# ChrisTho23/DrakeGPT

Hardware: AMD Instinct MI355X
Metric: training tokens/sec (fwd+bwd+AdamW) (higher is better)
Workload: dtype bf16; 1 GPU; TransformerLM_scaled: V=80 C=384 T=256 heads=6 layers=6 dropout=0.2; fwd+bwd+AdamW; hipGraph=on; batch_per_gpu=64, global_batch=64, seq_len=256, parallelism=dp1, dp_gradient_buckets=1, params=10800464

## Files before the change

drakegpt_amd/csrc/chain.hip:

```cpp
#include "common.h"
#include <stdlib.h>

typedef __attribute__((address_space(1))) const void* gptr_t;
typedef __attribute__((address_space(3))) void* lptr_t;

#define CH_C 384
#define CH_ROWS 64
#define CH_STAGE_B 24576
#define CH_STAGE_A 4096
#define CH_STAGE (CH_STAGE_B + CH_STAGE_A)
#define CH_NST 4
#define CH_ARES (CH_NST * CH_STAGE)
#define CH_KS (CH_C / 32)

struct ChainP {
    const char* o;
    const float* x;
    const char* wproj; const float* bproj;
    float* x1;
    const float* ln2w; const float* ln2b; float* mean2; float* rstd2; bf16_t* h2;
    const char* w1; const float* b1; bf16_t* f; unsigned char* bits;
    const char* w2; const float* b2;
    float* x2; bf16_t* x2b;
    const float* ln1w; const float* ln1b; float* mean1; float* rstd1; bf16_t* h1;
    const char* wqkv; bf16_t* qkv;
    int M, n_blocks;
    float eps;
    const uint32_t* rng; uint32_t site_proj, site_ffn, thr; float inv_keep; int drop;
    int stagger;
    unsigned long long* stamps;
    int dbg;
};

__device__ __forceinline__ void ch_wait_vm(int n) {
    switch (n) {
        case 6: asm volatile("s_waitcnt vmcnt(6)" ::: "memory"); break;
        case 7: asm volatile("s_waitcnt vmcnt(7)" ::: "memory"); break;
        case 12: asm volatile("s_waitcnt vmcnt(12)" ::: "memory"); break;
        case 13: asm volatile("s_waitcnt vmcnt(13)" ::: "memory"); break;
        case 14: asm volatile("s_waitcnt vmcnt(14)" ::: "memory"); break;
        case 8: asm volatile("s_waitcnt vmcnt(8)" ::: "memory"); break;
        case 18: asm volatile("s_waitcnt vmcnt(18)" ::: "memory"); break;
        case 20: asm volatile("s_waitcnt vmcnt(20)" ::: "memory"); break;
        default: asm volatile("s_waitcnt vmcnt(0)" ::: "memory"); break;
    }
}

template <int MODE>
__global__ __launch_bounds__(768) void block_chain_fwd_kernel(ChainP p) {
    constexpr int C = CH_C, KS = CH_KS;
    constexpr bool HAS_PROJ = MODE == 0 || MODE == 1 || MODE == 3, HAS_FFN1 = MODE == 0 || MODE == 1;
    constexpr bool HAS_FFN2 = MODE == 0 || MODE == 1 || MODE == 4, HAS_QKV = MODE == 0 || MODE == 2;
    constexpr bool LN_FFN2 = MODE == 0 || MODE == 4;
    constexpr int O_FFN1 = HAS_PROJ ? KS : 0, O_FFN2 = O_FFN1 + (HAS_FFN1 ? 4 * KS : 0), Q0 = O_FFN2 + (HAS_FFN2 ? 4 * KS : 0);
    constexpr int S = Q0 + (HAS_QKV ? 3 * KS : 0);
    __shared__ __attribute__((aligned(16))) char lds[CH_ARES + 6 * 8192];
    const int tid = threadIdx.x, lane = tid & 63, wave = __builtin_amdgcn_readfirstlane(tid >> 6);
    const bool loader = wave >= 8;
    if (p.stagger > 0) {
        const int grp = ((int)blockIdx.x >> 3) & 3;
        for (int i = 0; i < grp * p.stagger; ++i) __builtin_amdgcn_s_sleep(1);
    }

    auto n_of = [&](int s) -> int {
        if (MODE == 4) return (s & 1) ? 6 : 8;
        return (HAS_FFN2 && s >= O_FFN2 && s < Q0) ? 7 : 6;
    };
    auto ln_after = [&](int s) -> bool { return (HAS_PROJ && s == O_FFN1 - 1) || (LN_FFN2 && s == Q0 - 1); };

    if (loader) {
        const int lw = wave - 8;
        const int prow = lane >> 3, slot = lane & 7;
        const int ls = slot ^ prow;
        const uint32_t voff = (uint32_t)(lw * 6144 + lane * 16);
        const uint32_t aoff = (uint32_t)((lw * 8 + prow + 32 * (ls >> 2)) * (4 * C * 2) + (ls & 3) * 16);
        for (int blk = blockIdx.x; blk < p.n_blocks; blk += gridDim.x) {
            const int64_t row0 = (int64_t)blk * CH_ROWS;
            const char* fblk = (const char*)p.f + row0 * (int64_t)(4 * C * 2);
            auto issue = [&](int s) {
                if (p.dbg == 3 && s >= CH_NST) return;
                const char* src;
                if (HAS_PROJ && s < O_FFN1) src = p.wproj + (int64_t)s * CH_STAGE_B;
                else if (HAS_FFN1 && s < O_FFN2) src = p.w1 + (int64_t)(s - O_FFN1) * CH_STAGE_B;
                else if (HAS_FFN2 && s < Q0) src = p.w2 + (int64_t)(s - O_FFN2) * CH_STAGE_B;
                else src = p.wqkv + (int64_t)(s - Q0) * CH_STAGE_B;
                char* buf = lds + (s & (CH_NST - 1)) * CH_STAGE;
#pragma unroll
                for (int i = 0; i < 6; ++i)
                    __builtin_amdgcn_global_load_lds((gptr_t)(src + voff + i * 1024), (lptr_t)(buf + lw * 6144 + i * 1024), 16, 0, 0);
                if (MODE == 4) {
                    if (!(s & 1)) {
                        const int u = s >> 1;
#pragma unroll
                        for (int j = 0; j < 2; ++j) {
                            const int pr = lw * 2 + j;
                            const char* src = fblk + (int64_t)(pr * 8 + prow) * (4 * C * 2) + u * 128 + ((slot ^ prow) << 4);
                            __builtin_amdgcn_global_load_lds((gptr_t)src, (lptr_t)(lds + CH_ARES + (u % 6) * 8192 + pr * 1024), 16, 0, 0);
                        }
                    }
                } else if (HAS_FFN2 && s >= O_FFN2 && s < Q0)
                    __builtin_amdgcn_global_load_lds((gptr_t)(fblk + (s - O_FFN2) * 64 + aoff), (lptr_t)(buf + CH_STAGE_B + lw * 1024), 16, 0, 0);
            };
            if (HAS_PROJ) {
                const int chunk_std = slot ^ prow;
#pragma unroll
                for (int j = 0; j < 12; ++j) {
                    const int idx = lw * 12 + j, tile = idx >> 3, pr = idx & 7;
                    const char* src = p.o + (row0 + pr * 8 + prow) * (int64_t)(C * 2) + tile * 128 + chunk_std * 16;
                    __builtin_amdgcn_global_load_lds((gptr_t)src, (lptr_t)(lds + CH_ARES + tile * 8192 + pr * 1024), 16, 0, 0);
                }
            }
            for (int s = 0; s < CH_NST; ++s) issue(s);
            if (MODE == 2) __builtin_amdgcn_s_barrier();
            ch_wait_vm(n_of(1) + n_of(2) + n_of(3));
            __builtin_amdgcn_s_barrier();
            if (p.dbg == 5) {
                for (int b = 0; b + 1 < S; ++b) {
                    __builtin_amdgcn_s_barrier();
                    if (ln_after(b)) __builtin_amdgcn_s_barrier();
                }
                if (ln_after(S - 1)) __builtin_amdgcn_s_barrier();
                __builtin_amdgcn_s_barrier();
                continue;
            }
            for (int b = 0; b + 1 < S; ++b) {
                int fly = 0;
                if (b + 2 < S) fly += n_of(b + 2);
                if (b + 3 < S) fly += n_of(b + 3);
                ch_wait_vm(fly);
                __builtin_amdgcn_s_barrier();
                if (b + CH_NST < S) issue(b + CH_NST);
                if (ln_after(b)) __builtin_amdgcn_s_barrier();
            }
            if (ln_after(S - 1)) __builtin_amdgcn_s_barrier();
            __builtin_amdgcn_s_barrier();
        }
        return;
    }

    const int wm = wave >> 2, wn = wave & 3;
    const int fr = lane & 15, fg = lane >> 4;
    f32x4 acc[2][6];
#pragma unroll
    for (int i = 0; i < 2; ++i)
#pragma unroll
        for (int j = 0; j < 6; ++j) acc[i][j] = (f32x4){0.f, 0.f, 0.f, 0.f};
    const int b_off = ((wn & 1) * 96 + fr) * 128 + ((((wn >> 1) * 4 + fg) ^ (fr & 7)) << 4);
    const int ar_off = CH_STAGE_B + fr * 128 + (((wm * 4 + fg) ^ (fr & 7)) << 4);
    const int res_row = wm * 32 + fr;
    const int a_off0 = CH_ARES + res_row * 128 + (((0 + fg) ^ (fr & 7)) << 4);
    const int a_off1 = CH_ARES + res_row * 128 + (((4 + fg) ^ (fr & 7)) << 4);
    auto read_B = [&](u32x4 (&fb)[6], int s) {
        const char* buf = lds + (s & (CH_NST - 1)) * CH_STAGE + b_off;
#pragma unroll
        for (int j = 0; j < 6; ++j) fb[j] = *(const u32x4*)(buf + j * 2048);
    };
    auto read_A_ring = [&](u32x4 (&fa)[2], int s) {
        const char* buf = lds + (s & (CH_NST - 1)) * CH_STAGE + ar_off;
#pragma unroll
        for (int i = 0; i < 2; ++i) fa[i] = *(const u32x4*)(buf + i * 2048);
    };
    auto read_A_res = [&](u32x4 (&fa)[2], int t) {
        const char* buf = lds + ((t >> 1) % 6) * 8192 + ((t & 1) ? a_off1 : a_off0);
#pragma unroll
        for (int i = 0; i < 2; ++i) fa[i] = *(const u32x4*)(buf + i * 2048);
    };
    auto mma = [&](const u32x4 (&fa)[2], const u32x4 (&fb)[6]) {
        if (p.dbg == 2) return;
#pragma unroll
        for (int i = 0; i < 2; ++i)
#pragma unroll
            for (int j = 0; j < 6; ++j)
                acc[i][j] = __builtin_amdgcn_mfma_f32_16x16x32_bf16(__builtin_bit_cast(bf16x8, fb[j]), __builtin_bit_cast(bf16x8, fa[i]), acc[i][j], 0, 0, 0);
    };
    uint32_t key_proj = 0, key_ffn = 0;
    if (p.drop) { key_proj = dg_site_key_dev(p.rng, p.site_proj); key_ffn = dg_site_key_dev(p.rng, p.site_ffn); }
    const int col_l = wn * 96 + (fg & 1) * 16 + (fg >> 1) * 8;
    auto opaque_lane = [&]() -> int { int l = lane; asm volatile("" : "+v"(l)); return l; };
    auto mad24 = [](int a, int b, int c) -> int { int r; asm("v_mad_u32_u24 %0, %1, %2, %3" : "=v"(r) : "v"(a), "s"(b), "v"(c)); return r; };

    auto take = [&](int i, int q, float (&v)[8]) {
#pragma unroll
        for (int e = 0; e < 4; ++e) {
            float a = acc[i][2 * q][e], b = acc[i][2 * q + 1][e];
            asm volatile("s_nop 1\n\tv_permlane16_swap_b32 %0, %1\n\ts_nop 1" : "+v"(a), "+v"(b));
            v[e] = a;
            v[4 + e] = b;
        }
        acc[i][2 * q] = (f32x4){0.f, 0.f, 0.f, 0.f};
        acc[i][2 * q + 1] = (f32x4){0.f, 0.f, 0.f, 0.f};
    };
    auto drop8 = [&](float (&v)[8], uint32_t key, int64_t row0, int rl, int col) {
        const uint32_t i0 = (uint32_t)row0 * (uint32_t)C + (uint32_t)mad24(rl, C, col);
        const uint32_t w2 = (i0 >> 1) * DG_WEYL;
#pragma unroll
        for (int e = 0; e < 8; e += 2) {
            const uint32_t h = dg_hash_w(key, w2 + (uint32_t)(e >> 1) * DG_WEYL);
            v[e] = dg_keep_lo(h, p.thr) ? v[e] * p.inv_keep : 0.f;
            v[e + 1] = dg_keep_hi(h, p.thr) ? v[e + 1] * p.inv_keep : 0.f;
        }
    };
    auto layernorm = [&](float (&xv)[2][3][8], float* scratch, int64_t row0, const float* gamma, const float* beta, float* mean_o,
                         float* rstd_o, bf16_t* y) {
        const int lo = opaque_lane(), fr = lo & 15, fg = lo >> 4, col_l = wn * 96 + (fg & 1) * 16 + (fg >> 1) * 8;
#pragma unroll
        for (int i = 0; i < 2; ++i) {
            float s = 0.f;
#pragma unroll
            for (int q = 0; q < 3; ++q)
#pragma unroll
                for (int e = 0; e < 8; ++e) s += xv[i][q][e];
            s += __shfl_xor(s, 16, 64);
            s += __shfl_xor(s, 32, 64);
            const float mw = s * (1.f / 96.f);
            float m2 = 0.f;
#pragma unroll
            for (int q = 0; q < 3; ++q)
#pragma unroll
                for (int e = 0; e < 8; ++e) { const float d = xv[i][q][e] - mw; m2 += d * d; }
            m2 += __shfl_xor(m2, 16, 64);
            m2 += __shfl_xor(m2, 32, 64);
            if (fg == 0) *(f32x2*)(scratch + ((wm * 32 + i * 16 + fr) * 4 + wn) * 2) = (f32x2){mw, m2};
        }
        __builtin_amdgcn_s_barrier();
        float mu[2], rs[2];
#pragma unroll
        for (int i = 0; i < 2; ++i) {
            const f32x4 a = *(const f32x4*)(scratch + (wm * 32 + i * 16 + fr) * 8), b = *(const f32x4*)(scratch + (wm * 32 + i * 16 + fr) * 8 + 4);
            const float m = ((a[0] + a[2]) + (b[0] + b[2])) * 0.25f;
            const float d0 = a[0] - m, d1 = a[2] - m, d2 = b[0] - m, d3 = b[2] - m;
            const float M2 = ((a[1] + a[3]) + (b[1] + b[3])) + 96.f * ((d0 * d0 + d1 * d1) + (d2 * d2 + d3 * d3));
            mu[i] = m;
            rs[i] = rsqrtf(M2 * (1.f / (float)C) + p.eps);
            if (wn == 0 && fg == 0) { mean_o[row0 + wm * 32 + i * 16 + fr] = m; rstd_o[row0 + wm * 32 + i * 16 + fr] = rs[i]; }
        }
#pragma unroll
        for (int q = 0; q < 3; ++q) {
            const int col = col_l + 32 * q;
            const f32x4 g0 = *(const f32x4*)(gamma + col), g1 = *(const f32x4*)(gamma + col + 4);
            const f32x4 b0 = *(const f32x4*)(beta + col), b1 = *(const f32x4*)(beta + col + 4);
#pragma unroll
            for (int i = 0; i < 2; ++i) {
                bf16x8 o;
#pragma unroll
                for (int e = 0; e < 4; ++e) {
                    o[e] = (bf16_t)((xv[i][q][e] - mu[i]) * rs[i] * g0[e] + b0[e]);
                    o[4 + e] = (bf16_t)((xv[i][q][4 + e] - mu[i]) * rs[i] * g1[e] + b1[e]);
                }
                const int rl = wm * 32 + i * 16 + fr;
                if (p.dbg != 6) *(bf16x8*)(y + row0 * C + mad24(rl, C, col)) = o;
                *(bf16x8*)(lds + CH_ARES + (col >> 6) * 8192 + rl * 128 + ((((col & 63) >> 3) ^ (rl & 7)) << 4)) = o;
            }
        }
    };
    auto residual_epilogue = [&](float (&xv)[2][3][8], int64_t row0, const float* bias, const float* res, uint32_t key, float* out32, bf16_t* out16) {
        const int lo = opaque_lane(), fr = lo & 15, fg = lo >> 4, col_l = wn * 96 + (fg & 1) * 16 + (fg >> 1) * 8;
        f32x4 bq[2][2], r[2][2][2];
        auto request = [&](int q) {
            const int col = col_l + 32 * q;
            bq[q & 1][0] = *(const f32x4*)(bias + col); bq[q & 1][1] = *(const f32x4*)(bias + col + 4);
#pragma unroll
            for (int i = 0; i < 2; ++i) {
                const float* rp = res + row0 * C + mad24(wm * 32 + i * 16 + fr, C, col);
                if (p.dbg == 7) { r[q & 1][i][0] = bq[q & 1][0]; r[q & 1][i][1] = bq[q & 1][1]; continue; }
                r[q & 1][i][0] = *(const f32x4*)rp; r[q & 1][i][1] = *(const f32x4*)(rp + 4);
            }
        };
        request(0);
#pragma unroll
        for (int q = 0; q < 3; ++q) {
            if (q + 1 < 3) request(q + 1);
            const int col = col_l + 32 * q;
#pragma unroll
            for (int i = 0; i < 2; ++i) {
                const int64_t row = row0 + wm * 32 + i * 16 + fr;
                float v[8];
                take(i, q, v);
#pragma unroll
                for (int e = 0; e < 4; ++e) { v[e] += bq[q & 1][0][e]; v[4 + e] += bq[q & 1][1][e]; }
                if (p.drop) drop8(v, key, row0, wm * 32 + i * 16 + fr, col);
#pragma unroll
                for (int e = 0; e < 4; ++e) { v[e] += r[q & 1][i][0][e]; v[4 + e] += r[q & 1][i][1][e]; }
                if (p.dbg == 6) {
                } else if (out32) {
                    float* op = out32 + row0 * C + mad24(wm * 32 + i * 16 + fr, C, col);
                    *(f32x4*)op = (f32x4){v[0], v[1], v[2], v[3]};
                    *(f32x4*)(op + 4) = (f32x4){v[4], v[5], v[6], v[7]};
                } else {
                    bf16x8 o;
#pragma unroll
                    for (int e = 0; e < 8; ++e) o[e] = (bf16_t)v[e];
                    *(bf16x8*)(out16 + row0 * C + mad24(wm * 32 + i * 16 + fr, C, col)) = o;
                }
#pragma unroll
                for (int e = 0; e < 8; ++e) xv[i][q][e] = v[e];
            }
        }
    };

    if (p.dbg != 11) {
        const int jx = (int)blockIdx.x >> 3, per = ((int)gridDim.x >> 3) ? ((int)gridDim.x >> 3) : 1;
        float w0 = 0.f, w1 = 0.f, w2 = 0.f, w3 = 0.f;
        auto warm = [&](float& dst, const char* base, int n_stages) {
            const int i = jx + per * tid;
            if (i < n_stages * (CH_STAGE_B / 128)) asm volatile("global_load_dword %0, %1, off" : "=v"(dst) : "v"(base + (int64_t)i * 128) : "memory");
        };
        if (HAS_PROJ) warm(w0, p.wproj, KS);
        if (HAS_FFN1) warm(w1, p.w1, 4 * KS);
        if (HAS_FFN2) warm(w2, p.w2, 4 * KS);
        if (HAS_QKV) warm(w3, p.wqkv, 3 * KS);
        asm volatile("s_waitcnt vmcnt(0)" : "+v"(w0), "+v"(w1), "+v"(w2), "+v"(w3) :: "memory");
    }
    auto stamp = [&](int k) {
        if (p.stamps && wave == 0) {
            const unsigned long long t = __builtin_amdgcn_s_memtime();
            if (lane == 0) p.stamps[(int64_t)blockIdx.x * 24 + k] = t;
        }
    };
    u32x4 fa0[2], fb0[6], fa1[2], fb1[6];
    for (int blk = blockIdx.x; blk < p.n_blocks; blk += gridDim.x) {
        const int64_t row0 = (int64_t)blk * CH_ROWS;
        int g = 0;
        if (MODE == 2) {
            float xv[2][3][8];
#pragma unroll
            for (int q = 0; q < 3; ++q)
#pragma unroll
                for (int i = 0; i < 2; ++i) {
                    const float* xp = p.x + row0 * C + mad24(wm * 32 + i * 16 + fr, C, col_l + 32 * q);
                    const f32x4 a = *(const f32x4*)xp, b = *(const f32x4*)(xp + 4);
#pragma unroll
                    for (int e = 0; e < 4; ++e) { xv[i][q][e] = a[e]; xv[i][q][4 + e] = b[e]; }
                }
            layernorm(xv, (float*)(lds + 0 * CH_STAGE + CH_STAGE_B), row0, p.ln1w, p.ln1b, p.mean1, p.rstd1, p.h1);
        }
        __builtin_amdgcn_s_barrier();
        auto pipe_barrier = [&]() {
            __builtin_amdgcn_sched_barrier(0);
            asm volatile("s_waitcnt lgkmcnt(0)" ::: "memory");
            __builtin_amdgcn_s_barrier();
            __builtin_amdgcn_sched_barrier(0);
        };
        auto piece = [&](int nstep, bool ring_a, bool next, bool a_after_barrier, bool drain = false) {
            read_B(fb0, g);
            if (!a_after_barrier) { if (ring_a) read_A_ring(fa0, g); else read_A_res(fa0, 0); }
            for (int t = 0; t < nstep; t += 2) {
                if (drain && t == nstep - 2 && p.dbg != 10) asm volatile("s_waitcnt vmcnt(0)" ::: "memory");
                if (t == 8) asm volatile("s_waitcnt vmcnt(0)" ::: "memory");
                pipe_barrier();
                if (t == 0 && a_after_barrier) read_A_res(fa0, 0);
                read_B(fb1, g + 1);
                if (ring_a) read_A_ring(fa1, g + 1); else read_A_res(fa1, t + 1);
                mma(fa0, fb0);
                ++g;
                if (t + 2 < nstep) {
                    pipe_barrier();
                    read_B(fb0, g + 1);
                    if (ring_a) read_A_ring(fa0, g + 1); else read_A_res(fa0, t + 2);
                } else if (next) {
                    pipe_barrier();
                }
                mma(fa1, fb1);
                ++g;
            }
            __builtin_amdgcn_sched_barrier(0);
            asm volatile("s_nop 15\n\ts_nop 3" ::: "memory");
            __builtin_amdgcn_sched_barrier(0);
        };
        stamp(0);
        if (HAS_PROJ) {
            piece(KS, false, HAS_FFN1, false, true);
            stamp(1);
            if (p.dbg == 4 || p.dbg == 5) __builtin_amdgcn_s_barrier();
            else {
                float xv[2][3][8];
                residual_epilogue(xv, row0, p.bproj, p.x, key_proj, p.x1, nullptr);
                layernorm(xv, (float*)(lds + (g & (CH_NST - 1)) * CH_STAGE + CH_STAGE_B), row0, p.ln2w, p.ln2b, p.mean2, p.rstd2, p.h2);
            }
        }
        stamp(2);
        if (HAS_FFN1) {
            for (int c = 0; c < 4; ++c) {
                piece(KS, false, true, c == 0);
                stamp(3 + 2 * c);
                if (p.dbg == 4 || p.dbg == 5) continue;
                const int lo = opaque_lane(), fr = lo & 15, fg = lo >> 4, col_l = wn * 96 + (fg & 1) * 16 + (fg >> 1) * 8;
                const int lane = lo;
                const int tile_lo = (blk >> 1) * (4 * C / 192) + c * 2 + (wn >> 1);
                const int wv = (((blk & 1) * 2 + wm) * 2 + (wn & 1));
                f32x4 bq[3][2];
#pragma unroll
                for (int q = 0; q < 3; ++q) {
                    const int col = c * C + col_l + 32 * q;
                    bq[q][0] = *(const f32x4*)(p.b1 + col); bq[q][1] = *(const f32x4*)(p.b1 + col + 4);
                }
#pragma unroll
                for (int q = 0; q < 3; ++q) {
                    const int col = c * C + col_l + 32 * q;
#pragma unroll
                    for (int i = 0; i < 2; ++i) {
                        const int64_t row = row0 + wm * 32 + i * 16 + fr;
                        float v[8];
                        take(i, q, v);
                        unsigned bm = 0;
                        bf16x8 o;
#pragma unroll
                        for (int e = 0; e < 8; ++e) {
                            v[e] = fmaxf(v[e] + (e < 4 ? bq[q][0][e] : bq[q][1][e - 4]), 0.f);
                            bm |= (v[e] > 0.f ? 1u : 0u) << e;
                            o[e] = (bf16_t)v[e];
                        }
                        if (p.dbg != 6) {
                            p.bits[((((int64_t)tile_lo * 8 + wv) * 3 + q) * 2 + i) * 64 + lane] = (unsigned char)bm;
                            *(bf16x8*)(p.f + row0 * (4 * C) + mad24(wm * 32 + i * 16 + fr, 4 * C, col)) = o;
                        }
                    }
                }
                stamp(4 + 2 * c);
            }
        }
        if (HAS_FFN2) {
            piece(4 * KS, MODE != 4, HAS_QKV, false, true);
            stamp(11);
            if (p.dbg == 4 || p.dbg == 5) { if (LN_FFN2) __builtin_amdgcn_s_barrier(); }
            else {
                float xv[2][3][8];
                residual_epilogue(xv, row0, p.b2, p.x1, key_ffn, MODE != 1 ? p.x2 : nullptr, p.x2b);
                if (LN_FFN2)
                    layernorm(xv, (float*)(lds + (g & (CH_NST - 1)) * CH_STAGE + CH_STAGE_B), row0, p.ln1w, p.ln1b, p.mean1, p.rstd1, p.h1);
            }
        }
        stamp(12);
        if (HAS_QKV) {
            for (int c = 0; c < 3; ++c) {
                piece(KS, false, c < 2, MODE == 0 && c == 0);
                stamp(13 + 2 * c);
                if (p.dbg == 4 || p.dbg == 5) continue;
                const int lo = opaque_lane(), fr = lo & 15, fg = lo >> 4, col_l = wn * 96 + (fg & 1) * 16 + (fg >> 1) * 8;
#pragma unroll
                for (int q = 0; q < 3; ++q) {
                    const int col = c * C + col_l + 32 * q;
#pragma unroll
                    for (int i = 0; i < 2; ++i) {
                        const int64_t row = row0 + wm * 32 + i * 16 + fr;
                        float v[8];
                        take(i, q, v);
                        bf16x8 o;
#pragma unroll
                        for (int e = 0; e < 8; ++e) o[e] = (bf16_t)v[e];
                        if (p.dbg != 6) *(bf16x8*)(p.qkv + row0 * (3 * C) + mad24(wm * 32 + i * 16 + fr, 3 * C, col)) = o;
                    }
                }
                stamp(14 + 2 * c);
            }
        }
        stamp(19);
        __builtin_amdgcn_s_barrier();
        stamp(20);
    }
}

struct PackOne { const unsigned short* src; unsigned short* dst; int N, K; int64_t ld; };
__global__ __launch_bounds__(256) void pack_chain_kernel(const int64_t* __restrict__ desc, int n_desc, PackOne one) {
    const unsigned short* src = one.src;
    unsigned short* dst = one.dst;
    int K = one.K;
    int64_t ld = one.ld;
    int k = blockIdx.x;
    if (desc) {
        int d = 0;
        for (int i = 1; i < n_desc; ++i)
            if ((int64_t)blockIdx.x >= desc[i * 6 + 4]) d = i;
        const int64_t* D = desc + d * 6;
        src = (const unsigned short*)D[0]; dst = (unsigned short*)D[1]; K = (int)D[3]; ld = D[5];
        k = (int)((int64_t)blockIdx.x - D[4]);
    }
    const int KT = K / 32, c = k / KT, t = k % KT;
#pragma unroll
    for (int u = 0; u < 6; ++u) {
        const int idx = threadIdx.x + 256 * u, line = idx >> 3, slot = idx & 7, ls = slot ^ (line & 7);
        const int row = c * 384 + line + 192 * (ls >> 2), col = t * 32 + 8 * (ls & 3);
        *(u32x4*)(dst + ((int64_t)k * 1536 + idx) * 8) = *(const u32x4*)(src + (int64_t)row * ld + col);
    }
}

extern "C" int dg_pack_chain_weights(const void* w, int64_t ld, void* packed, int N, int K, void* stream) {
    if (!w || !packed || N <= 0 || K <= 0 || N % 384 || K % 32 || ld < K || ld % 8 || !dg_aligned16(w) || !dg_aligned16(packed)) return DG_ERR_ARG;
    PackOne one{(const unsigned short*)w, (unsigned short*)packed, N, K, ld};
    hipLaunchKernelGGL(pack_chain_kernel, dim3((N / 384) * (K / 32)), dim3(256), 0, (hipStream_t)stream, (const int64_t*)nullptr, 0, one);
    DG_LAUNCH_CHECK();
    return DG_OK;
}

extern "C" int dg_pack_chain_weights_batched(const int64_t* desc, int n_desc, int total_stages, void* stream) {
    if (!desc || n_desc <= 0 || total_stages <= 0) return DG_ERR_ARG;
    PackOne one{nullptr, nullptr, 0, 0, 0};
    hipLaunchKernelGGL(pack_chain_kernel, dim3(total_stages), dim3(256), 0, (hipStream_t)stream, desc, n_desc, one);
    DG_LAUNCH_CHECK();
    return DG_OK;
}

__global__ __launch_bounds__(256) void l2_warm_kernel(const char* __restrict__ p, int64_t n_lines, float* __restrict__ sink) {
    const int j = (int)blockIdx.x >> 3, per = (int)gridDim.x >> 3;
    float acc = 0.f;
    for (int64_t i = (int64_t)j * 256 + threadIdx.x; i < n_lines; i += (int64_t)per * 256) acc += *(const float*)(p + i * 128);
    if (acc == 123.456f && sink) sink[0] = acc;
}

extern "C" int dg_l2_warm(const void* p, int64_t bytes, void* stream) {
    if (!p || bytes <= 0 || (((uintptr_t)p) & 127)) return DG_ERR_ARG;
    hipLaunchKernelGGL(l2_warm_kernel, dim3(256), dim3(256), 0, (hipStream_t)stream, (const char*)p, bytes / 128, (float*)nullptr);
    DG_LAUNCH_CHECK();
    return DG_OK;
}

static int ch_num_cus() {
    static const int v = [] {
        int dev = 0, n = 256;
        if (hipGetDevice(&dev) == hipSuccess) {
            int x = 0;
            if (hipDeviceGetAttribute(&x, hipDeviceAttributeMultiprocessorCount, dev) == hipSuccess && x > 0) n = x;
        }
        return n;
    }();
    return v;
}

extern "C" int dg_block_chain_supported(int M, int C) { return M > 0 && M % CH_ROWS == 0 && C == CH_C; }

static unsigned long long* g_chain_stamps = nullptr;
extern "C" void dg_debug_set_chain_fwd_stamps(void* q) { g_chain_stamps = (unsigned long long*)q; }

extern "C" int dg_block_chain_fwd(const dg_block_chain_args* a, void* stream) {
    if (!a || !dg_block_chain_supported(a->M, a->C)) return DG_ERR_ARG;
    if (a->mode < 0 || a->mode > 4) return DG_ERR_ARG;
    if (a->dropout_p < 0.f || a->dropout_p >= 1.f) return DG_ERR_ARG;
    const int m = a->mode;
    const bool has_proj = m == 0 || m == 1 || m == 3, has_ffn1 = m == 0 || m == 1, has_ffn2 = m == 0 || m == 1 || m == 4;
    const bool has_qkv = m == 0 || m == 2, ln1 = m == 0 || m == 2 || m == 4;
    auto al = [](const void* q) { return q && dg_aligned16(q); };
    if (!al(a->x) && m != 4) return DG_ERR_ARG;
    if (has_proj && (!al(a->o) || !al(a->wproj) || !al(a->bproj) || !al(a->x1) || !al(a->ln2w) || !al(a->ln2b) || !a->mean2 || !a->rstd2 || !al(a->h2)))
        return DG_ERR_ARG;
    if (has_ffn1 && (!al(a->w1) || !al(a->b1) || !a->sign_bits ||
                     a->sign_bits_bytes < (int64_t)((a->M + 127) / 128) * (4 * a->C / 192) * (128 * 192 / 8))) return DG_ERR_ARG;
    if (has_ffn2 && (!al(a->f) || !al(a->x1) || !al(a->w2) || !al(a->b2) || (m == 1 ? !al(a->x2_bf16) : !al(a->x2)))) return DG_ERR_ARG;
    if (ln1 && (!al(a->ln1w) || !al(a->ln1b) || !a->mean1 || !a->rstd1 || !al(a->h1))) return DG_ERR_ARG;
    if (has_qkv && (!al(a->wqkv) || !al(a->qkv))) return DG_ERR_ARG;
    ChainP p;
    p.o = (const char*)a->o; p.x = a->x; p.wproj = (const char*)a->wproj; p.bproj = a->bproj; p.x1 = a->x1;
    p.ln2w = a->ln2w; p.ln2b = a->ln2b; p.mean2 = a->mean2; p.rstd2 = a->rstd2; p.h2 = (bf16_t*)a->h2;
    p.w1 = (const char*)a->w1; p.b1 = a->b1; p.f = (bf16_t*)a->f; p.bits = a->sign_bits;
    p.w2 = (const char*)a->w2; p.b2 = a->b2; p.x2 = a->x2; p.x2b = (bf16_t*)a->x2_bf16;
    p.ln1w = a->ln1w; p.ln1b = a->ln1b; p.mean1 = a->mean1; p.rstd1 = a->rstd1; p.h1 = (bf16_t*)a->h1;
    p.wqkv = (const char*)a->wqkv; p.qkv = (bf16_t*)a->qkv;
    p.M = a->M; p.n_blocks = a->M / CH_ROWS; p.eps = a->eps;
    p.drop = (a->dropout_p > 0.f && a->rng_state) ? 1 : 0;
    p.rng = a->rng_state; p.site_proj = a->site_proj; p.site_ffn = a->site_ffn;
    p.thr = dg_drop_threshold(a->dropout_p); p.inv_keep = 1.f / (1.f - a->dropout_p);
    { static const int dbg = [] { const char* e = getenv("DG_CHAIN_DBG"); return e ? atoi(e) : 0; }(); p.dbg = dbg; }
    p.stamps = g_chain_stamps;
    { static const int st = [] { const char* e = getenv("DG_CHAIN_STAGGER"); return e ? atoi(e) : 0; }(); p.stagger = st; }
    const dim3 grid(p.n_blocks < ch_num_cus() ? p.n_blocks : ch_num_cus()), block(768);
    hipStream_t s = (hipStream_t)stream;
    switch (m) {
        case 0: hipLaunchKernelGGL(block_chain_fwd_kernel<0>, grid, block, 0, s, p); break;
        case 1: hipLaunchKernelGGL(block_chain_fwd_kernel<1>, grid, block, 0, s, p); break;
        case 2: hipLaunchKernelGGL(block_chain_fwd_kernel<2>, grid, block, 0, s, p); break;
        case 3: hipLaunchKernelGGL(block_chain_fwd_kernel<3>, grid, block, 0, s, p); break;
        default: hipLaunchKernelGGL(block_chain_fwd_kernel<4>, grid, block, 0, s, p); break;
    }
    DG_LAUNCH_CHECK();
    return DG_OK;
}
```

Measured before the change: 6.942 million tokens/s.

## Stage bias and LayerNorm vectors in LDS via loader waves; specialize wait counts

Loader waves now also copy the bias, gamma and beta vectors into spare LDS regions with async global-to-LDS loads, and the compute waves read them from LDS instead of global memory in the epilogues and layernorm. The loader pipeline is restructured into per-segment loops with constant vmcnt waits and tracked in-flight counts, replacing the per-stage n_of computation. The weight pack kernel gets a path for even K-tile counts that coalesces global reads across pairs of tiles. This trades more complex vmcnt bookkeeping, where a miscount could race, for fewer global loads and less scalar overhead on the compute waves.

```diff
diff --git a/drakegpt_amd/csrc/chain.hip b/drakegpt_amd/csrc/chain.hip
--- a/drakegpt_amd/csrc/chain.hip
+++ b/drakegpt_amd/csrc/chain.hip
@@ -62,10 +62,7 @@
         for (int i = 0; i < grp * p.stagger; ++i) __builtin_amdgcn_s_sleep(1);
     }
 
-    auto n_of = [&](int s) -> int {
-        if (MODE == 4) return (s & 1) ? 6 : 8;
-        return (HAS_FFN2 && s >= O_FFN2 && s < Q0) ? 7 : 6;
-    };
+    constexpr int VEC_BIAS = 0 * CH_STAGE + CH_STAGE_B + 2048, VEC_GB = 1 * CH_STAGE + CH_STAGE_B;
     auto ln_after = [&](int s) -> bool { return (HAS_PROJ && s == O_FFN1 - 1) || (LN_FFN2 && s == Q0 - 1); };
 
     if (loader) {
@@ -77,29 +74,64 @@
         for (int blk = blockIdx.x; blk < p.n_blocks; blk += gridDim.x) {
             const int64_t row0 = (int64_t)blk * CH_ROWS;
             const char* fblk = (const char*)p.f + row0 * (int64_t)(4 * C * 2);
-            auto issue = [&](int s) {
-                if (p.dbg == 3 && s >= CH_NST) return;
+            auto vec1 = [&](const float* v) {
+                int l = lane; asm volatile("" : "+v"(l));
+                if (l < 24) __builtin_amdgcn_global_load_lds((gptr_t)(v + lw * 96 + l * 4), (lptr_t)(lds + VEC_BIAS + lw * 384), 16, 0, 0);
+            };
+            auto vec2 = [&](const float* gm, const float* bt) {
+                int l = lane; asm volatile("" : "+v"(l));
+                if (l < 48)
+                    __builtin_amdgcn_global_load_lds((gptr_t)(l < 24 ? gm + lw * 96 + l * 4 : bt + lw * 96 + (l - 24) * 4),
+                                                     (lptr_t)(lds + VEC_GB + lw * 768), 16, 0, 0);
+            };
+            auto issue_a = [&](int s, char* buf) {
+                if (MODE != 4) {
+                    __builtin_amdgcn_global_load_lds((gptr_t)(fblk + (s - O_FFN2) * 64 + aoff), (lptr_t)(buf + CH_STAGE_B + lw * 1024), 16, 0, 0);
+                    return;
+                }
+                if (s & 1) return;
+                const int u = s >> 1;
+#pragma unroll
+                for (int j = 0; j < 2; ++j) {
+                    const int pr = lw * 2 + j;
+                    const char* src = fblk + (int64_t)(pr * 8 + prow) * (4 * C * 2) + u * 128 + ((slot ^ prow) << 4);
+                    __builtin_amdgcn_global_load_lds((gptr_t)src, (lptr_t)(lds + CH_ARES + (u % 6) * 8192 + pr * 1024), 16, 0, 0);
+                }
+            };
+            auto issue = [&](int s) -> int {
+                const bool off = p.dbg == 3 && s >= CH_NST;
+                int n = 6;
                 const char* src;
+                char* buf = lds + (s & (CH_NST - 1)) * CH_STAGE;
                 if (HAS_PROJ && s < O_FFN1) src = p.wproj + (int64_t)s * CH_STAGE_B;
-                else if (HAS_FFN1 && s < O_FFN2) src = p.w1 + (int64_t)(s - O_FFN1) * CH_STAGE_B;
-                else if (HAS_FFN2 && s < Q0) src = p.w2 + (int64_t)(s - O_FFN2) * CH_STAGE_B;
-                else src = p.wqkv + (int64_t)(s - Q0) * CH_STAGE_B;
-                char* buf = lds + (s & (CH_NST - 1)) * CH_STAGE;
-#pragma unroll
-                for (int i = 0; i < 6; ++i)
-                    __builtin_amdgcn_global_load_lds((gptr_t)(src + voff + i * 1024), (lptr_t)(buf + lw * 6144 + i * 1024), 16, 0, 0);
-                if (MODE == 4) {
-                    if (!(s & 1)) {
-                        const int u = s >> 1;
-#pragma unroll
-                        for (int j = 0; j < 2; ++j) {
-                            const int pr = lw * 2 + j;
-                            const char* src = fblk + (int64_t)(pr * 8 + prow) * (4 * C * 2) + u * 128 + ((slot ^ prow) << 4);
-                            __builtin_amdgcn_global_load_lds((gptr_t)src, (lptr_t)(lds + CH_ARES + (u % 6) * 8192 + pr * 1024), 16, 0, 0);
-                        }
-                    }
-                } else if (HAS_FFN2 && s >= O_FFN2 && s < Q0)
-                    __builtin_amdgcn_global_load_lds((gptr_t)(fblk + (s - O_FFN2) * 64 + aoff), (lptr_t)(buf + CH_STAGE_B + lw * 1024), 16, 0, 0);
+                else if (HAS_FFN1 && s < O_FFN2) {
+                    const int r = s - O_FFN1;
+                    src = p.w1 + (int64_t)r * CH_STAGE_B;
+                    if (r == 0) { if (!off) vec1(p.bproj); ++n; }
+                    else if (r == 1) { if (!off) vec2(p.ln2w, p.ln2b); ++n; }
+                    else if (r == KS || r == 2 * KS || r == 3 * KS) { if (!off) vec1(p.b1 + (r / KS - 1) * C); ++n; }
+                } else if (HAS_FFN2 && s < Q0) {
+                    src = p.w2 + (int64_t)(s - O_FFN2) * CH_STAGE_B;
+                    n += MODE != 4 ? 1 : (s & 1) ? 0 : 2;
+                    if (!off) issue_a(s, buf);
+                } else {
+                    src = p.wqkv + (int64_t)(s - Q0) * CH_STAGE_B;
+                    if (MODE == 0 && s == Q0) { if (!off) vec1(p.b2); ++n; }
+                    else if (MODE == 0 && s == Q0 + 1) { if (!off) vec2(p.ln1w, p.ln1b); ++n; }
+                }
+                asm volatile("" : "+s"(src));
+                if (!off) {
+#pragma unroll
+                    for (int i = 0; i < 6; ++i)
+                        __builtin_amdgcn_global_load_lds((gptr_t)(src + voff + i * 1024), (lptr_t)(buf + lw * 6144 + i * 1024), 16, 0, 0);
+                }
+                if ((MODE == 2 || MODE == 3 || MODE == 4) && s == 0) {
+                    if (MODE == 3) { vec1(p.bproj); ++n; }
+                    if (MODE == 4) { vec1(p.b2); ++n; }
+                    if (MODE == 3) vec2(p.ln2w, p.ln2b); else vec2(p.ln1w, p.ln1b);
+                    ++n;
+                }
+                return n;
             };
             if (HAS_PROJ) {
                 const int chunk_std = slot ^ prow;
@@ -110,9 +142,14 @@
                     __builtin_amdgcn_global_load_lds((gptr_t)src, (lptr_t)(lds + CH_ARES + tile * 8192 + pr * 1024), 16, 0, 0);
                 }
             }
-            for (int s = 0; s < CH_NST; ++s) issue(s);
-            if (MODE == 2) __builtin_amdgcn_s_barrier();
-            ch_wait_vm(n_of(1) + n_of(2) + n_of(3));
+            issue(0);
+            const int n1 = issue(1);
+            int n_prev = issue(2), n_last = issue(3);
+            if (MODE == 2) {
+                ch_wait_vm(n1 + n_prev + n_last);
+                __builtin_amdgcn_s_barrier();
+            }
+            ch_wait_vm(n1 + n_prev + n_last);
             __builtin_amdgcn_s_barrier();
             if (p.dbg == 5) {
                 for (int b = 0; b + 1 < S; ++b) {
@@ -123,14 +160,52 @@
                 __builtin_amdgcn_s_barrier();
                 continue;
             }
-            for (int b = 0; b + 1 < S; ++b) {
-                int fly = 0;
-                if (b + 2 < S) fly += n_of(b + 2);
-                if (b + 3 < S) fly += n_of(b + 3);
-                ch_wait_vm(fly);
+            auto adv = [&](int b, int n_issued) {
+                n_prev = n_last;
+                n_last = n_issued;
+                if (ln_after(b)) {
+                    ch_wait_vm(n_prev + n_last);
+                    __builtin_amdgcn_s_barrier();
+                }
+            };
+            auto seg = [&](int lo, int hi, const char* w, bool ffn2) {
+#pragma unroll
+                for (int k = 0; k < 6; ++k) {
+                    const int s = lo + k;
+                    if (s < CH_NST) continue;
+                    ch_wait_vm(n_prev + n_last);
+                    __builtin_amdgcn_s_barrier();
+                    adv(s - CH_NST, issue(s));
+                }
+                const char* base = w + (int64_t)6 * CH_STAGE_B;
+#pragma nounroll
+                for (int s = lo + 6; s < hi; ++s, base += CH_STAGE_B) {
+                    if (ffn2) asm volatile("s_waitcnt vmcnt(14)" ::: "memory"); else asm volatile("s_waitcnt vmcnt(12)" ::: "memory");
+                    __builtin_amdgcn_s_barrier();
+                    if (p.dbg == 3) continue;
+                    char* buf = lds + (s & (CH_NST - 1)) * CH_STAGE;
+                    const char* src = base;
+                    asm volatile("" : "+s"(src));
+#pragma unroll
+                    for (int i = 0; i < 6; ++i)
+                        __builtin_amdgcn_global_load_lds((gptr_t)(src + voff + i * 1024), (lptr_t)(buf + lw * 6144 + i * 1024), 16, 0, 0);
+                    if (ffn2) issue_a(s, buf);
+                }
+                n_prev = ffn2 ? (MODE == 4 ? 8 : 7) : 6;
+                n_last = ffn2 ? (MODE == 4 ? 6 : 7) : 6;
+            };
+            if (HAS_PROJ) seg(0, O_FFN1, p.wproj, false);
+            if (HAS_FFN1) {
+#pragma unroll
+                for (int c = 0; c < 4; ++c) seg(O_FFN1 + c * KS, O_FFN1 + (c + 1) * KS, p.w1 + (int64_t)c * KS * CH_STAGE_B, false);
+            }
+            if (HAS_FFN2) seg(O_FFN2, Q0, p.w2, true);
+            if (HAS_QKV) seg(Q0, S, p.wqkv, false);
+#pragma unroll
+            for (int b = S - CH_NST; b + 1 < S; ++b) {
+                ch_wait_vm(n_prev + n_last);
                 __builtin_amdgcn_s_barrier();
-                if (b + CH_NST < S) issue(b + CH_NST);
-                if (ln_after(b)) __builtin_amdgcn_s_barrier();
+                adv(b, 0);
             }
             if (ln_after(S - 1)) __builtin_amdgcn_s_barrier();
             __builtin_amdgcn_s_barrier();
@@ -200,8 +275,7 @@
             v[e + 1] = dg_keep_hi(h, p.thr) ? v[e + 1] * p.inv_keep : 0.f;
         }
     };
-    auto layernorm = [&](float (&xv)[2][3][8], float* scratch, int64_t row0, const float* gamma, const float* beta, float* mean_o,
-                         float* rstd_o, bf16_t* y) {
+    auto layernorm = [&](float (&xv)[2][3][8], float* scratch, int64_t row0, float* mean_o, float* rstd_o, bf16_t* y) {
         const int lo = opaque_lane(), fr = lo & 15, fg = lo >> 4, col_l = wn * 96 + (fg & 1) * 16 + (fg >> 1) * 8;
 #pragma unroll
         for (int i = 0; i < 2; ++i) {
@@ -237,8 +311,9 @@
 #pragma unroll
         for (int q = 0; q < 3; ++q) {
             const int col = col_l + 32 * q;
-            const f32x4 g0 = *(const f32x4*)(gamma + col), g1 = *(const f32x4*)(gamma + col + 4);
-            const f32x4 b0 = *(const f32x4*)(beta + col), b1 = *(const f32x4*)(beta + col + 4);
+            const char* gb = lds + VEC_GB + wn * 768 + (col - wn * 96) * 4;
+            const f32x4 g0 = *(const f32x4*)gb, g1 = *(const f32x4*)(gb + 16);
+            const f32x4 b0 = *(const f32x4*)(gb + 384), b1 = *(const f32x4*)(gb + 400);
 #pragma unroll
             for (int i = 0; i < 2; ++i) {
                 bf16x8 o;
@@ -258,7 +333,8 @@
         f32x4 bq[2][2], r[2][2][2];
         auto request = [&](int q) {
             const int col = col_l + 32 * q;
-            bq[q & 1][0] = *(const f32x4*)(bias + col); bq[q & 1][1] = *(const f32x4*)(bias + col + 4);
+            if (bias) { bq[q & 1][0] = *(const f32x4*)(bias + col); bq[q & 1][1] = *(const f32x4*)(bias + col + 4); }
+            else { bq[q & 1][0] = *(const f32x4*)(lds + VEC_BIAS + col * 4); bq[q & 1][1] = *(const f32x4*)(lds + VEC_BIAS + col * 4 + 16); }
 #pragma unroll
             for (int i = 0; i < 2; ++i) {
                 const float* rp = res + row0 * C + mad24(wm * 32 + i * 16 + fr, C, col);
@@ -332,7 +408,7 @@
 #pragma unroll
                     for (int e = 0; e < 4; ++e) { xv[i][q][e] = a[e]; xv[i][q][4 + e] = b[e]; }
                 }
-            layernorm(xv, (float*)(lds + 0 * CH_STAGE + CH_STAGE_B), row0, p.ln1w, p.ln1b, p.mean1, p.rstd1, p.h1);
+            layernorm(xv, (float*)(lds + 0 * CH_STAGE + CH_STAGE_B), row0, p.mean1, p.rstd1, p.h1);
         }
         __builtin_amdgcn_s_barrier();
         auto pipe_barrier = [&]() {
@@ -374,8 +450,8 @@
             if (p.dbg == 4 || p.dbg == 5) __builtin_amdgcn_s_barrier();
             else {
                 float xv[2][3][8];
-                residual_epilogue(xv, row0, p.bproj, p.x, key_proj, p.x1, nullptr);
-                layernorm(xv, (float*)(lds + (g & (CH_NST - 1)) * CH_STAGE + CH_STAGE_B), row0, p.ln2w, p.ln2b, p.mean2, p.rstd2, p.h2);
+                residual_epilogue(xv, row0, nullptr, p.x, key_proj, p.x1, nullptr);
+                layernorm(xv, (float*)(lds + (g & (CH_NST - 1)) * CH_STAGE + CH_STAGE_B), row0, p.mean2, p.rstd2, p.h2);
             }
         }
         stamp(2);
@@ -391,8 +467,9 @@
                 f32x4 bq[3][2];
 #pragma unroll
                 for (int q = 0; q < 3; ++q) {
-                    const int col = c * C + col_l + 32 * q;
-                    bq[q][0] = *(const f32x4*)(p.b1 + col); bq[q][1] = *(const f32x4*)(p.b1 + col + 4);
+                    const int col = col_l + 32 * q;
+                    if (c < 3) { bq[q][0] = *(const f32x4*)(lds + VEC_BIAS + col * 4); bq[q][1] = *(const f32x4*)(lds + VEC_BIAS + col * 4 + 16); }
+                    else { bq[q][0] = *(const f32x4*)(p.b1 + c * C + col); bq[q][1] = *(const f32x4*)(p.b1 + c * C + col + 4); }
                 }
 #pragma unroll
                 for (int q = 0; q < 3; ++q) {
@@ -425,9 +502,9 @@
             if (p.dbg == 4 || p.dbg == 5) { if (LN_FFN2) __builtin_amdgcn_s_barrier(); }
             else {
                 float xv[2][3][8];
-                residual_epilogue(xv, row0, p.b2, p.x1, key_ffn, MODE != 1 ? p.x2 : nullptr, p.x2b);
+                residual_epilogue(xv, row0, MODE == 1 ? p.b2 : nullptr, p.x1, key_ffn, MODE != 1 ? p.x2 : nullptr, p.x2b);
                 if (LN_FFN2)
-                    layernorm(xv, (float*)(lds + (g & (CH_NST - 1)) * CH_STAGE + CH_STAGE_B), row0, p.ln1w, p.ln1b, p.mean1, p.rstd1, p.h1);
+                    layernorm(xv, (float*)(lds + (g & (CH_NST - 1)) * CH_STAGE + CH_STAGE_B), row0, p.mean1, p.rstd1, p.h1);
             }
         }
         stamp(12);
@@ -476,6 +553,18 @@
         k = (int)((int64_t)blockIdx.x - D[4]);
     }
     const int KT = K / 32, c = k / KT, t = k % KT;
+    if (!(KT & 1)) {
+        const int half = t & 1, t0 = t - half;
+        const int64_t k0 = k - half;
+#pragma unroll
+        for (int u = 0; u < 6; ++u) {
+            const int idx = threadIdx.x + 256 * u, line = 96 * half + (idx >> 4), hi = (idx >> 3) & 1, j = idx & 7;
+            const int slot = (hi * 4 + (j & 3)) ^ (line & 7);
+            const int row = c * 384 + line + 192 * hi, col = t0 * 32 + 8 * j;
+            *(u32x4*)(dst + ((k0 + (j >> 2)) * 1536 + line * 8 + slot) * 8) = *(const u32x4*)(src + (int64_t)row * ld + col);
+        }
+        return;
+    }
 #pragma unroll
     for (int u = 0; u < 6; ++u) {
         const int idx = threadIdx.x + 256 * u, line = idx >> 3, slot = idx & 7, ls = slot ^ (line & 7);
```

Result: faster. 7.113 million tokens/s (median of 6 runs) (+2.5%).
